# LJacksonPan/RaTrack

Hardware: AMD Instinct MI355X
Metric: radar frame-pairs/sec (backbone forward, eval) at B=64,N=256 per GPU (higher is better)
Workload: dtype f32 (2xfp16 split MFMA: three fp16 products per fp32 product, fp32 accumulate, power-of-two scales per matrix and position); 1 GPU; Track4D.backbone forward, B=64 frame-pairs x N=256 points per GPU, S=512 centroids, eval-mode BN, random-init weights, hipGraph=True, batches in flight=4; global_batch=64, parallelism=replicas x1 (no collective on the forward path)

## Files before the change

### ratrack_amd/csrc/fused_split.hip

```cpp
#include "rtk_common.h"
#include "rtk_fused.h"
#include "split_mfma.h"

namespace {

#ifndef SP_NW
#define SP_NW 4
#endif
#ifndef SP_F
#define SP_F 32
#endif
constexpr int CV_F = 32;

__global__ __launch_bounds__(256) void pack_split_kernel(int cout, int cin, const float *__restrict__ w, int transposed, u4v *__restrict__ out,
                                                         float *__restrict__ inv_scale) {
    __shared__ unsigned s_m[4];
    float m = 0.f;
    const f4 *w4 = reinterpret_cast<const f4 *>(w);
    for (int i = threadIdx.x; i < cout * cin / 4; i += 256) {
        const f4 t = w4[i];
        m = __builtin_fmaxf(__builtin_fmaxf(m, __builtin_fabsf(t.x)), __builtin_fabsf(t.y));
        m = __builtin_fmaxf(__builtin_fmaxf(m, __builtin_fabsf(t.z)), __builtin_fabsf(t.w));
    }
    unsigned mb = __float_as_uint(m);
// ... 103 lines not shown
                const unsigned bit = (a[4 * v + q][r] > 0.f ? 1u : 0u) << (4 * ((2 * v + (q >> 1)) & 7) + r);
                if (v < 4) m[q & 1].x |= bit; else m[q & 1].y |= bit;
            }
}
__device__ __forceinline__ unsigned split_mask_bits(const uint2 (&m)[2], int v, int q) {
    return ((v < 4 ? m[q & 1].x : m[q & 1].y) >> (4 * ((2 * v + (q >> 1)) & 7))) & 15u;
}

__device__ __forceinline__ f4 *cv_at(float *base, unsigned byte_off) { return reinterpret_cast<f4 *>(reinterpret_cast<char *>(base) + byte_off); }
__device__ __forceinline__ const f4 *cv_at(const float *base, unsigned byte_off) {
    return reinterpret_cast<const f4 *>(reinterpret_cast<const char *>(base) + byte_off);
}

__device__ __forceinline__ void wn_hidden(const WnSplit &W, float dx, float dy, float dz, float (&t2)[8]) {
    float t1[8];
#pragma unroll
    for (int o = 0; o < 8; ++o) {
        float a = __fmaf_rn(ldc(W.wa + o), dx, 0.f);
        a = __fmaf_rn(ldc(W.wa + 16 + o), dy, a);
        a = __fmaf_rn(ldc(W.wa + 32 + o), dz, a);
        t1[o] = fmaxf(__fadd_rn(a, ldc(W.wa + 48 + o)), 0.f);
    }
#pragma unroll
    for (int o = 0; o < 8; ++o) {
        float a = ldc(W.bb + o);
#pragma unroll
        for (int c = 0; c < 8; ++c) a = __fmaf_rn(ldc(W.wb + (16 * (c >> 2) + o) * 4 + (c & 3)), t1[c], a);
        t2[o] = fmaxf(a, 0.f);
    }
}
struct WnBlock {
    f16v bias;
    float w[4];
};
__device__ __forceinline__ WnBlock wn_block(const WnSplit &W, int v, int hh, int col) {
    WnBlock k;
    k.bias = split_bias(W.bc, v, hh);
    const int ch = 32 * v + col;
    const float *wr = W.wc + ((ch >> 4) * 64 + (ch & 15)) * 4;
#pragma unroll
    for (int st = 0; st < 4; ++st) {
        const int kk = 2 * st + hh;
        k.w[st] = ldc(wr + 64 * (kk >> 2) + (kk & 3));
    }
    return k;
}
__device__ __forceinline__ f16v wn_pre(const WnBlock &k, int hh, const float (&t2)[8]) {
    f16v w = k.bias;
#pragma unroll
    for (int st = 0; st < 4; ++st) w = mfma_f32x2(k.w[st], hh ? t2[2 * st + 1] : t2[2 * st], w);
    return w;
}
__device__ __forceinline__ float rtk_hidden_inf() {
    float v;
    asm volatile("s_mov_b32 %0, 0x7f800000" : "=s"(v));
    return v;
}
__device__ __forceinline__ float relu1(float x, float inf) { return __builtin_amdgcn_fmed3f(x, 0.f, inf); }
__device__ __forceinline__ f4 relu_med4(f4 t, float inf) { return (f4){relu1(t.x, inf), relu1(t.y, inf), relu1(t.z, inf), relu1(t.w, inf)}; }

constexpr int CV_ROWS_F4 = 32 * 32;
struct CvRowsRequest {
    const char *p2;
    f4 *rows;
    int nbrow;
    unsigned lanepart;
    int sub;
    __device__ __forceinline__ CvRowsRequest(const float *p2_, f4 *rows_, int nbrow_, int half, int lane)
        : p2(reinterpret_cast<const char *>(p2_)), rows(rows_), nbrow(nbrow_), lanepart(512u * half + (unsigned)(((lane & 31) ^ (lane >> 5)) << 4)), sub(lane >> 5) {}
    template <int T>
    __device__ __forceinline__ void one() const {
        const int r0 = __builtin_amdgcn_readlane(nbrow, 2 * T), r1 = __builtin_amdgcn_readlane(nbrow, 2 * T + 1);
        const unsigned off = ((unsigned)(sub ? r1 : r0) << 10) + (lanepart ^ (unsigned)(((2 * T) & 15) << 4));
        __builtin_amdgcn_global_load_lds((const __attribute__((address_space(1))) void *)(p2 + off),
                                         (__attribute__((address_space(3))) void *)(rows + T * 64), 16, 0, 0);
    }
    template <int... T>
    __device__ __forceinline__ void all(std::integer_sequence<int, T...>) const { (one<T>(), ...); }
};
template <int HALF>
__device__ __forceinline__ void cv_rows_request(const float *p2, int nbrow, f4 *rows, int lane) {
    asm volatile("s_waitcnt lgkmcnt(0)" ::: "memory");
    CvRowsRequest(p2, rows, nbrow, HALF, lane).all(std::make_integer_sequence<int, 16>{});
}
template <bool SAVE>
struct CvLayer2Side {
    StoreRowsSide st;
    CvRowsRequest rq;
    template <int GI>
    __device__ __forceinline__ void at(const f4 (&h)[32]) const {
        if constexpr (SAVE) st.template at<GI>(h);
        constexpr int per_chunk = CV_F / SPLIT_GF, ig = split_issue_groups(CV_F), g = GI % per_chunk, n = (GI / per_chunk) * ig + g;
        if constexpr (g < ig && 3 * n < 16) {
            rq.template one<3 * n>();
            if constexpr (3 * n + 1 < 16) rq.template one<3 * n + 1>();
            if constexpr (3 * n + 2 < 16) rq.template one<3 * n + 2>();
        }
    }
};
template <int HALF>
__device__ __forceinline__ void cv_rows_read(const f4 *rows, int col, int hh, f4 (&h)[32]) {
#pragma unroll
    for (int e = 0; e < 16; ++e) h[16 * HALF + e] = rows[col * 32 + ((2 * e + hh) ^ (col & 15))];
}
template <int K>
__device__ __forceinline__ f4 add_row_bcast(const f4 q, const f4 r) {
    f4 o;
    asm("s_nop 1\n"
        "v_add_f32_dpp %0, %4, %8 row_newbcast:%12 row_mask:0xf bank_mask:0xf\n"
        "v_add_f32_dpp %1, %5, %9 row_newbcast:%12 row_mask:0xf bank_mask:0xf\n"
        "v_add_f32_dpp %2, %6, %10 row_newbcast:%12 row_mask:0xf bank_mask:0xf\n"
        "v_add_f32_dpp %3, %7, %11 row_newbcast:%12 row_mask:0xf bank_mask:0xf"
        : "=&v"(o.x), "=&v"(o.y), "=&v"(o.z), "=&v"(o.w)
        : "v"(q.x), "v"(q.y), "v"(q.z), "v"(q.w), "v"(r.x), "v"(r.y), "v"(r.z), "v"(r.w), "n"(K));
    return o;
}
template <int K>
__device__ __forceinline__ f4 mul_row_bcast(const f4 q, const f4 r) {
    f4 o;
    asm("s_nop 1\n"
        "v_mul_f32_dpp %0, %4, %8 row_newbcast:%12 row_mask:0xf bank_mask:0xf\n"
        "v_mul_f32_dpp %1, %5, %9 row_newbcast:%12 row_mask:0xf bank_mask:0xf\n"
        "v_mul_f32_dpp %2, %6, %10 row_newbcast:%12 row_mask:0xf bank_mask:0xf\n"
        "v_mul_f32_dpp %3, %7, %11 row_newbcast:%12 row_mask:0xf bank_mask:0xf"
        : "=&v"(o.x), "=&v"(o.y), "=&v"(o.z), "=&v"(o.w)
        : "v"(q.x), "v"(q.y), "v"(q.z), "v"(q.w), "v"(r.x), "v"(r.y), "v"(r.z), "v"(r.w), "n"(K));
    return o;
}
__device__ __forceinline__ f4 add4_rn(const f4 a, const f4 b) {
    return (f4){__fadd_rn(a.x, b.x), __fadd_rn(a.y, b.y), __fadd_rn(a.z, b.z), __fadd_rn(a.w, b.w)};
}
template <int V0, int V1>
__device__ __forceinline__ void cv_layer1_blocks(const CvSplitParams &P, const f4 q0, const f4 q1, float b0, float b1, int hh, int col, float kinf, f4 (&h)[32]) {
    static_assert(V1 <= 8, "eight 32-channel blocks");
    auto block = [&](auto vc) {
        constexpr int v = decltype(vc)::value;
        f16v c;
        auto slot = [&](auto qc) {
            constexpr int q = decltype(qc)::value, e = 4 * v + q;
            const f4 t = add_row_bcast<e & 15>(e < 16 ? q0 : q1, h[e]);
            c[4 * q] = t.x; c[4 * q + 1] = t.y; c[4 * q + 2] = t.z; c[4 * q + 3] = t.w;
        };
        slot(std::integral_constant<int, 0>{}); slot(std::integral_constant<int, 1>{});
        slot(std::integral_constant<int, 2>{}); slot(std::integral_constant<int, 3>{});
        const int ch = 32 * v + col;
        const float *wr = P.wd + (ch >> 4) * 64 + (ch & 15);
        c = mfma_f32x2(ldc(wr + 16 * hh), b0, c);
        c = mfma_f32x2(ldc(wr + 16 * (2 + hh)), b1, c);
#pragma unroll
        for (int q = 0; q < 4; ++q) h[4 * v + q] = leaky_med4((f4){c[4 * q], c[4 * q + 1], c[4 * q + 2], c[4 * q + 3]}, kinf);
    };
    block(std::integral_constant<int, V0>{}); block(std::integral_constant<int, V0 + 1>{});
    block(std::integral_constant<int, V0 + 2>{}); block(std::integral_constant<int, V0 + 3>{});
}

#ifndef CV_FWD_VGPRS
#define CV_FWD_VGPRS 448
#endif
template <bool SAVE>
__global__ __launch_bounds__(64 * SP_NW) __attribute__((amdgpu_waves_per_eu(1, 1), amdgpu_num_vgpr(CV_FWD_VGPRS)))
void cost_volume_split_kernel(const CvSplitParams P) {
    const float kinf = rtk_hidden_inf();
    __shared__ __attribute__((aligned(16))) f4 s_w[2 * CV_F * 64];
    __shared__ __attribute__((aligned(16))) f4 s_rows[SP_NW * CV_ROWS_F4];
    const int lane = threadIdx.x & 63, wave = __builtin_amdgcn_readfirstlane(threadIdx.x >> 6), hh = lane >> 5, col = lane & 31, pp = col >> 4,
              j = col & 15;
    f4 *rows = s_rows + wave * CV_ROWS_F4;
    constexpr int PPW = 2 * SP_NW;
    const int groups = (P.n1 + PPW - 1) / PPW;
    const bool flat = P.gx > 0;
    const int xcd = blockIdx.x & 7, t0 = flat ? (int)(blockIdx.x >> 3) : (int)blockIdx.x, tstep = flat ? P.gx >> 3 : (int)gridDim.x;
    const int ntiles = flat ? (P.samples >> 3) * groups : groups;
    auto locate = [&](int t, int &b_, int &G_) {
        if (flat) { const int sk = t / groups; b_ = sk * 8 + xcd; G_ = t - sk * groups; }
        else { b_ = blockIdx.y; G_ = t; }
    };
    int b, bx;
    locate(t0 < ntiles ? t0 : 0, b, bx);
    WStreamA<SP_NW, CV_F, 2 * SPLIT_NF> ws;
    ws.start_parts(P.blob, s_w, wave, lane);
    const float wi2 = ldc(P.wsc), wi3 = ldc(P.wsc + 1);
    int pt = bx * PPW + 2 * wave + pp;
    bool valid = pt < P.n1;
    long i = (long)b * P.n1 + (valid ? pt : P.n1 - 1);
    long nb = 0;
    float dx = 0.f, dy = 0.f, dz = 0.f;
    f4 q0 = {0.f, 0.f, 0.f, 0.f}, q1 = q0;
    if (t0 < ntiles) {
        nb = (long)b * P.n2 + (long)P.knn[i * 16 + j];
        cv_rows_request<0>(P.p2, (int)nb, rows, lane);
        q0 = ldc4(P.p1 + i * 256 + 4 * hh + 8 * j); q1 = ldc4(P.p1 + i * 256 + 4 * hh + 8 * (16 + j));
        if (P.st) { q0 = add4_rn(q0, ldc4(P.st + b * 256 + 4 * hh + 8 * j)); q1 = add4_rn(q1, ldc4(P.st + b * 256 + 4 * hh + 8 * (16 + j))); }
        dx = __fsub_rn(P.xyz2[nb * 3], P.xyz1[i * 3]); dy = __fsub_rn(P.xyz2[nb * 3 + 1], P.xyz1[i * 3 + 1]);
        dz = __fsub_rn(P.xyz2[nb * 3 + 2], P.xyz1[i * 3 + 2]);
    }
    for (int t = t0; t < ntiles; t += tstep) {
        asm volatile("" ::: "memory");
        const bool more = t + tstep < ntiles;
        int bn, Gn;
        locate(more ? t + tstep : t, bn, Gn);
        const int ptn = Gn * PPW + 2 * wave + pp;
        const bool validn = ptn < P.n1;
        const long in_ = (long)bn * P.n1 + (validn ? ptn : P.n1 - 1);
        long knn_next = 0;
        if (more) knn_next = (long)P.knn[in_ * 16 + j];
        f4 h[32];
        float t2[8];
        {
            const float b0 = hh ? dy : dx, b1 = hh ? 0.f : dz;
            cv_rows_read<0>(rows, col, hh, h);
            cv_rows_request<1>(P.p2, (int)nb, rows, lane);
            cv_layer1_blocks<0, 4>(P, q0, q1, b0, b1, hh, col, kinf, h);
            wn_hidden(P.wn, dx, dy, dz, t2);
            __builtin_amdgcn_sched_barrier(0);
            cv_rows_read<1>(rows, col, hh, h);
            cv_layer1_blocks<4, 8>(P, q0, q1, b0, b1, hh, col, kinf, h);
        }
        const long nbn = (long)bn * P.n2 + knn_next;
        const long pos = i * 16 + j;
        const unsigned ro = (unsigned)pos * 1024u + 16u * hh;
        if (SAVE && valid) {
            uint2 m[2];
            split_sign_masks(h, m);
            P.mk1[pos * 4 + hh] = m[0];
            P.mk1[pos * 4 + 2 + hh] = m[1];
        }
        f16v acc[SPLIT_VB];
        f4 bq[2][8];
        LaneScale sc = lane_scale32(h);
        if (SAVE && P.amax) tensor_amax_update(P.amax, sc.mb);
        split_layer<0>(ws, h, sc.s, acc, SidePair<CvLayer2Side<SAVE>, BiasSide>{{StoreRowsSide{P.sv1, ro, valid}, CvRowsRequest(P.p2, rows, (int)nbn, 0, lane)},
                                                                              BiasSide{P.bias2 + 4 * hh, bq}});
        float c = sc.inv * wi2;
        split_epilogue(acc, P.bias2 + 4 * hh, bq, [&](int e, f4 a, f4 b) { h[e] = leaky_med4(scale_bias4(a, c, b), kinf); });
        if (SAVE && valid) {
            uint2 m[2];
            split_sign_masks(h, m);
            P.mk2[pos * 4 + hh] = m[0];
            P.mk2[pos * 4 + 2 + hh] = m[1];
        }
        sc = lane_scale32(h);
        if (SAVE && P.amax) tensor_amax_update(P.amax + 1, sc.mb);
        if (SAVE) split_layer<SPLIT_NF>(ws, h, sc.s, acc, SidePair<StoreRowsSide, BiasSide>{StoreRowsSide{P.sv2, ro, valid}, BiasSide{P.bias3 + 4 * hh, bq}});
        else split_layer<SPLIT_NF>(ws, h, sc.s, acc, BiasSide{P.bias3 + 4 * hh, bq});
        ws.sync();
        c = sc.inv * wi3;
        split_epilogue(acc, P.bias3 + 4 * hh, bq, [&](int e, f4 a, f4 b) { h[e] = leaky_med4(scale_bias4(a, c, b), kinf); });
        if (SAVE && valid) {
#pragma unroll
            for (int e = 0; e < 32; ++e) *cv_at(P.sv3, ro + 32u * e) = h[e];
        }
        WnBlock wk = wn_block(P.wn, 0, hh, col);
        float *o = P.out + i * P.out_pitch + 4 * hh;
        f16v wpre = wn_pre(wk, hh, t2);
        wk = wn_block(P.wn, 1, hh, col);
        auto out_block = [&](int v) {
            const f16v w = wpre;
            if (v + 1 < SPLIT_VB) wpre = wn_pre(wk, hh, t2);
            if (v + 2 < SPLIT_VB) wk = wn_block(P.wn, v + 2, hh, col);
            f4 r[4];
#pragma unroll
            for (int q = 0; q < 4; ++q)
#pragma unroll
                for (int e = 0; e < 4; ++e) r[q][e] = relu1(w[4 * q + e], kinf) * h[4 * v + q][e];
            const f4 t = row_sum16_transpose4(r[0], r[1], r[2], r[3]);
            if (valid && (j & 3) == 0) *reinterpret_cast<f4 *>(o + 32 * v + 8 * (2 * ((j >> 3) & 1) + ((j >> 2) & 1))) = t;
        };
        out_block(0);
        out_block(1);
        float cn[6] = {0.f, 0.f, 0.f, 0.f, 0.f, 0.f};
        f4 q0n = q0, q1n = q1, s0n = q0, s1n = q1;
        if (more) {
#pragma unroll
            for (int c = 0; c < 3; ++c) { cn[c] = ldc(P.xyz2 + nbn * 3 + c); cn[3 + c] = ldc(P.xyz1 + in_ * 3 + c); }
            q0n = ldc4(P.p1 + in_ * 256 + 4 * hh + 8 * j); q1n = ldc4(P.p1 + in_ * 256 + 4 * hh + 8 * (16 + j));
        }
        if (more && P.st) { s0n = ldc4(P.st + bn * 256 + 4 * hh + 8 * j); s1n = ldc4(P.st + bn * 256 + 4 * hh + 8 * (16 + j)); }
#pragma unroll
        for (int v = 2; v < SPLIT_VB; ++v) out_block(v);
        pt = ptn; valid = validn; i = in_; nb = nbn; q0 = q0n; q1 = q1n;
        if (P.st) { q0 = add4_rn(q0n, s0n); q1 = add4_rn(q1n, s1n); }
        dx = __fsub_rn(cn[0], cn[3]); dy = __fsub_rn(cn[1], cn[4]); dz = __fsub_rn(cn[2], cn[5]);
    }
    ws.finish();
}

struct CvSplitBwdParams {
    CvSplitParams f;
    const float *dout;
    int dout_pitch;
    const float *a3;
    const uint2 *mk1, *mk2;
    float *dz1, *dz2, *dz3, *dq3, *d4, *dp1, *dpd, *dt2, *dbrows;
};

__device__ __forceinline__ f4 leaky_grad_bits4(f4 d, unsigned bits) {
    return (f4){(bits & 1u) ? d.x : 0.1f * d.x, (bits & 2u) ? d.y : 0.1f * d.y, (bits & 4u) ? d.z : 0.1f * d.z, (bits & 8u) ? d.w : 0.1f * d.w};
}

__global__ __launch_bounds__(64 * SP_NW) __attribute__((amdgpu_waves_per_eu(1, 1))) void cost_volume_bwd_split_kernel(const CvSplitBwdParams Q) {
    const float kinf = rtk_hidden_inf();
    __shared__ __attribute__((aligned(16))) f4 s_w[2 * SP_F * 64];
    __shared__ float s_wct[128 * 64];
    const CvSplitParams &P = Q.f;
    const int lane = threadIdx.x & 63, wave = __builtin_amdgcn_readfirstlane(threadIdx.x >> 6), hh = lane >> 5, col = lane & 31, pp = col >> 4,
              j = col & 15;
    const int jq = 2 * ((j >> 3) & 1) + ((j >> 2) & 1);
    for (int e = threadIdx.x; e < 128 * 64; e += 64 * SP_NW) {
        const int l = e & 63, st = e >> 6, o = l & 31, ch = 32 * (st >> 4) + 8 * ((st >> 2) & 3) + 4 * (l >> 5) + (st & 3);
        s_wct[e] = o < 8 ? P.wn.wc[((ch >> 4) * 64 + (o >> 2) * 16 + (ch & 15)) * 4 + (o & 3)] : 0.f;
    }
    int b, bx, nbx;
    rtk_decode_block(P.gx, b, bx, nbx);
    constexpr int PPW = 2 * SP_NW;
    const int groups = (P.n1 + PPW - 1) / PPW;
    WStreamA<SP_NW, SP_F, 2 * SPLIT_NF> ws;
    ws.start_parts(P.blob, s_w, wave, lane);
    const float wi3 = ldc(P.wsc), wi2 = ldc(P.wsc + 1);
    int pt = bx * PPW + 2 * wave + pp;
    bool valid = pt < P.n1;
    long i = (long)b * P.n1 + (valid ? pt : P.n1 - 1);
    float dx = 0.f, dy = 0.f, dz = 0.f;
    if (bx < groups) {
        const long nb = (long)b * P.n2 + (long)P.knn[i * 16 + j];
        dx = __fsub_rn(P.xyz2[nb * 3], P.xyz1[i * 3]); dy = __fsub_rn(P.xyz2[nb * 3 + 1], P.xyz1[i * 3 + 1]);
        dz = __fsub_rn(P.xyz2[nb * 3 + 2], P.xyz1[i * 3 + 2]);
    }
    for (int G = bx; G < groups; G += nbx) {
        asm volatile("" ::: "memory");
        const long pos = i * 16 + j;
        const unsigned ro = (unsigned)pos * 1024u + 16u * hh;
        if (valid && hh == 0) *reinterpret_cast<f4 *>(Q.d4 + pos * 4) = (f4){dx, dy, dz, 1.0f};
        uint2 m2[2] = {Q.mk2[pos * 4 + hh], Q.mk2[pos * 4 + 2 + hh]}, m1[2] = {Q.mk1[pos * 4 + hh], Q.mk1[pos * 4 + 2 + hh]};
        f4 h[32];
#pragma unroll
        for (int e = 0; e < 32; ++e) h[e] = *cv_at(Q.a3, ro + 32u * e);
        float t2[8];
        WnBlock wk = wn_block(P.wn, 0, hh, col);
        const float *dor = Q.dout + i * Q.dout_pitch + 4 * hh;
        const f4 dq0 = ldc4(dor + 8 * j), dq1 = ldc4(dor + 8 * (16 + j));
        wn_hidden(P.wn, dx, dy, dz, t2);
        f16v dt2;
#pragma unroll
        for (int e = 0; e < 16; ++e) dt2[e] = 0.f;
        f16v wpre = wn_pre(wk, hh, t2);
        wk = wn_block(P.wn, 1, hh, col);
        auto block_a = [&](auto vc) {
            constexpr int v = decltype(vc)::value;
            const f16v w = wpre;
            if constexpr (v + 1 < SPLIT_VB) wpre = wn_pre(wk, hh, t2);
            if constexpr (v + 2 < SPLIT_VB) wk = wn_block(P.wn, v + 2, hh, col);
            f4 zs[4];
            auto slot = [&](auto qc) {
                constexpr int q = decltype(qc)::value, e = 4 * v + q;
                const f4 a = h[e];
                f4 wv;
#pragma unroll
                for (int r = 0; r < 4; ++r) wv[r] = relu1(w[4 * q + r], kinf);
                const f4 da = mul_row_bcast<e & 15>(e < 16 ? dq0 : dq1, a);
                const f4 t = mul_row_bcast<e & 15>(e < 16 ? dq0 : dq1, wv);
                f4 qq, z;
#pragma unroll
                for (int r = 0; r < 4; ++r) {
                    qq[r] = wv[r] > 0.f ? da[r] : 0.f;
                    z[r] = a[r] > 0.f ? t[r] : 0.1f * t[r];
                    dt2 = mfma_f32x2(s_wct[(16 * v + 4 * q + r) * 64 + lane], qq[r], dt2);
                }
                h[e] = z;
                zs[q] = z;
                if (valid) *cv_at(Q.dq3, ro + 32u * e) = qq;
            };
            slot(std::integral_constant<int, 0>{}); slot(std::integral_constant<int, 1>{});
            slot(std::integral_constant<int, 2>{}); slot(std::integral_constant<int, 3>{});
            if (Q.dbrows) {
                const f4 r = row_sum16_transpose4(zs[0], zs[1], zs[2], zs[3]);
                if (valid && (j & 3) == 0) *reinterpret_cast<f4 *>(Q.dbrows + i * 512 + 32 * v + 8 * jq + 4 * hh) = r;
            }
        };
        block_a(std::integral_constant<int, 0>{}); block_a(std::integral_constant<int, 1>{}); block_a(std::integral_constant<int, 2>{});
        block_a(std::integral_constant<int, 3>{}); block_a(std::integral_constant<int, 4>{}); block_a(std::integral_constant<int, 5>{});
        block_a(std::integral_constant<int, 6>{}); block_a(std::integral_constant<int, 7>{});
        if (valid) *reinterpret_cast<f4 *>(Q.dt2 + pos * 8 + 4 * hh) = (f4){dt2[0], dt2[1], dt2[2], dt2[3]};
        f16v acc[SPLIT_VB];
        LaneScale sc = lane_scale32(h);
        if (P.amax) tensor_amax_update(P.amax, sc.mb);
        split_layer<0>(ws, h, sc.s, acc, StoreRowsSide{Q.dz3, ro, valid});
        float c = sc.inv * wi3;
#pragma unroll
        for (int v = 0; v < SPLIT_VB; ++v) {
#pragma unroll
            for (int q = 0; q < 4; ++q) h[4 * v + q] = leaky_grad_bits4(acc_slot(acc, 4 * v + q) * c, split_mask_bits(m2, v, q));
            if (Q.dbrows) {
                const f4 r = row_sum16_transpose4(h[4 * v], h[4 * v + 1], h[4 * v + 2], h[4 * v + 3]);
                if (valid && (j & 3) == 0) *reinterpret_cast<f4 *>(Q.dbrows + i * 512 + 256 + 32 * v + 8 * jq + 4 * hh) = r;
            }
        }
        sc = lane_scale32(h);
        if (P.amax) tensor_amax_update(P.amax + 1, sc.mb);
        split_layer<SPLIT_NF>(ws, h, sc.s, acc, StoreRowsSide{Q.dz2, ro, valid});
        ws.sync();
        c = sc.inv * wi2;
        const int Gn = G + nbx;
        const bool more = Gn < groups;
        const int ptn = Gn * PPW + 2 * wave + pp;
        const bool validn = ptn < P.n1;
        const long in_ = (long)b * P.n1 + (validn ? ptn : P.n1 - 1);
        long knn_next = 0;
        if (more) knn_next = (long)P.knn[in_ * 16 + j];
        float dxn = 0.f, dyn = 0.f, dzn = 0.f;
        float *dpr = Q.dp1 + i * 256 + 4 * hh;
        float *dpd = Q.dpd + i * 768 + 4 * hh;
#pragma unroll
        for (int v = 0; v < SPLIT_VB; ++v) {
            if (v == 2 && more) {
                const long nbn = (long)b * P.n2 + knn_next;
                dxn = __fsub_rn(P.xyz2[nbn * 3], P.xyz1[in_ * 3]); dyn = __fsub_rn(P.xyz2[nbn * 3 + 1], P.xyz1[in_ * 3 + 1]);
                dzn = __fsub_rn(P.xyz2[nbn * 3 + 2], P.xyz1[in_ * 3 + 2]);
            }
            f4 r[4];
#pragma unroll
            for (int q = 0; q < 4; ++q) {
                r[q] = leaky_grad_bits4(acc_slot(acc, 4 * v + q) * c, split_mask_bits(m1, v, q));
                if (valid) *cv_at(Q.dz1, ro + 32u * (4 * v + q)) = r[q];
            }
            const f4 s0 = row_sum16_transpose4(r[0], r[1], r[2], r[3]);
            const f4 sx = row_sum16_transpose4(r[0] * dx, r[1] * dx, r[2] * dx, r[3] * dx);
            const f4 sy = row_sum16_transpose4(r[0] * dy, r[1] * dy, r[2] * dy, r[3] * dy);
            const f4 sz = row_sum16_transpose4(r[0] * dz, r[1] * dz, r[2] * dz, r[3] * dz);
            if (valid && (j & 3) == 0) {
                *reinterpret_cast<f4 *>(dpr + 32 * v + 8 * jq) = s0;
                *reinterpret_cast<f4 *>(dpd + 32 * v + 8 * jq) = sx;
                *reinterpret_cast<f4 *>(dpd + 256 + 32 * v + 8 * jq) = sy;
// ... 284 lines not shown
```

### ratrack_amd/csrc/split_mfma.h

```cpp
#pragma once
#include "fused_common.h"

typedef float f16v __attribute__((ext_vector_type(16)));

__device__ __forceinline__ f16v mfma_h(u4v a, u4v b, f16v c) {
    return __builtin_amdgcn_mfma_f32_32x32x16_f16(__builtin_bit_cast(h8v, a), __builtin_bit_cast(h8v, b), c, 0, 0, 0);
}

__device__ __forceinline__ f16v mfma_bf(u4v a, u4v b, f16v c) {
    return __builtin_amdgcn_mfma_f32_32x32x16_bf16(__builtin_bit_cast(bf8v, a), __builtin_bit_cast(bf8v, b), c, 0, 0, 0);
}

__device__ __forceinline__ LaneScale lane_scale32_of(float m) {
    const unsigned mb = __float_as_uint(m);
    const auto r = __builtin_amdgcn_permlane32_swap(mb, mb, false, false);
    return lane_scale_of(r[0] > r[1] ? r[0] : r[1]);
}
template <int N>
__device__ __forceinline__ LaneScale lane_scale32(const f4 (&h)[N]) { return lane_scale32_of(abs_max_f4(h)); }

template <int W>
__device__ __forceinline__ void split2_word_of(const f4 x0, const f4 x1, float s, u4v (&b)[2]) {
    const float xa = W < 2 ? x0[2 * W] : x1[2 * W - 4], xb = W < 2 ? x0[2 * W + 1] : x1[2 * W - 3];
    const SplitWord w = split2_word(xa, xb, s);
    b[0][W] = w.h; b[1][W] = w.l;
}

constexpr int SPLIT_GF = 4;
constexpr int split_issue_groups(int F) { return F >= 16 ? F / 16 : 1; }
constexpr int SPLIT_KS = 16;
constexpr int SPLIT_VB = 8;
constexpr int SPLIT_NF = SPLIT_KS * SPLIT_VB * 2;

template <int NW, int F, int NF>
struct WStreamA : WStream<NW, F, NF> {
    using Base = WStream<NW, F, NF>;
    unsigned rd;
    unsigned next_off;
    __device__ __forceinline__ void set_rd() {
        rd = (unsigned)(size_t)(__attribute__((address_space(3))) void *)(this->lds) + (unsigned)((this->buf * F) * 64 + this->lane) * 16u;
        const int nxt = this->cur + 1 == Base::NCHUNKS ? 0 : this->cur + 1;
        next_off = (unsigned)nxt * (unsigned)(F * 1024);
    }
    __device__ __forceinline__ void start(const f4 *blob_, f4 *lds_, int wave_, int lane_) { Base::start(blob_, lds_, wave_, lane_); set_rd(); }
    __device__ __forceinline__ void next() { Base::next(); set_rd(); }
    __device__ __forceinline__ void sync() {
        asm volatile("s_waitcnt vmcnt(0)" ::: "memory");
        __syncthreads();
        this->buf ^= 1;
        this->cur = this->cur + 1 == Base::NCHUNKS ? 0 : this->cur + 1;
        asm volatile("" : "+s"(this->cur));
        set_rd();
    }
    template <int K, int PARTS>
    __device__ __forceinline__ void issue_part() {
        static_assert(NF % F == 0, "whole chunks only");
        const char *base = this->blob + next_off;
#pragma unroll
        for (int i = K; i < (F + NW - 1) / NW; i += PARTS) {
            const int f = this->wave + i * NW;
            if (F % NW == 0 || f < F)
                __builtin_amdgcn_global_load_lds((const __attribute__((address_space(1))) void *)(base + (size_t)i * NW * 1024 + this->lane_off),
                                                 (__attribute__((address_space(3))) void *)(this->lds + ((this->buf ^ 1) * F + f) * 64), 16, 0, 0);
        }
    }
    __device__ __forceinline__ void start_parts(const f4 *blob_, f4 *lds_, int wave_, int lane_) {
        this->lds = lds_; this->wave = wave_; this->lane = lane_;
        this->blob = reinterpret_cast<const char *>(blob_);
        this->lane_off = (unsigned)(wave_ * 64 + lane_) * 16u;
        this->cur = 0; this->buf = 0;
        Base::issue(0, 0);
        asm volatile("s_waitcnt vmcnt(0)" ::: "memory");
        __syncthreads();
        set_rd();
    }
    template <int FI>
    __device__ __forceinline__ f4 frag_async() const {
        f4 r;
        asm volatile("ds_read_b128 %0, %1 offset:%2" : "=v"(r) : "v"(rd), "n"(FI * 1024));
        return r;
    }
};

template <int OUTSTANDING>
__device__ __forceinline__ void lds_wait(f4 (&c)[SPLIT_GF]) {
    asm volatile("s_waitcnt lgkmcnt(%4)" : "+v"(c[0]), "+v"(c[1]), "+v"(c[2]), "+v"(c[3]) : "n"(OUTSTANDING));
}

struct NoSide {
    template <int GI>
    __device__ __forceinline__ void at(const f4 (&)[32]) const {}
};
struct StoreRowsSide {
    float *base;
    unsigned ro;
    bool valid;
    template <int GI>
    __device__ __forceinline__ void at(const f4 (&h)[32]) const {
        if constexpr ((GI & 1) == 0) {
            if (valid) *reinterpret_cast<f4 *>(reinterpret_cast<char *>(base) + (ro + 32u * (GI / 2))) = h[GI / 2];
        }
    }
};
__device__ __forceinline__ float ldc(const float *p) { return *(const __attribute__((address_space(4))) float *)p; }
__device__ __forceinline__ f4 ldc4(const float *p) { return *(const __attribute__((address_space(4))) f4 *)p; }

__device__ __forceinline__ f4 bias_slot(const float *bias4hh, int e) {
    return *reinterpret_cast<const f4 *>(bias4hh + 32 * (e >> 2) + 8 * (e & 3));
}
struct BiasSide {
    const float *bias;
    f4 (&bq)[2][8];
    template <int GI>
    __device__ __forceinline__ void at(const f4 (&)[32]) const {
        constexpr int NG = SPLIT_KS * (SPLIT_VB / 2);
        if constexpr (GI >= NG - 4) {
            bq[0][2 * (GI - (NG - 4))] = bias_slot(bias, 2 * (GI - (NG - 4)));
            bq[0][2 * (GI - (NG - 4)) + 1] = bias_slot(bias, 2 * (GI - (NG - 4)) + 1);
        }
    }
};
template <class Emit>
__device__ __forceinline__ void split_epilogue(const f16v (&acc)[SPLIT_VB], const float *bias4hh, f4 (&bq)[2][8], Emit &&emit) {
#pragma unroll
    for (int k = 0; k < 4; ++k) {
        if (k < 3) {
#pragma unroll
            for (int e = 0; e < 8; ++e) bq[(k + 1) & 1][e] = bias_slot(bias4hh, 8 * (k + 1) + e);
        }
#pragma unroll
        for (int e = 0; e < 8; ++e) {
            const int v = (8 * k + e) >> 2, q = e & 3;
            emit(8 * k + e, (f4){acc[v][4 * q], acc[v][4 * q + 1], acc[v][4 * q + 2], acc[v][4 * q + 3]}, bq[k & 1][e]);
        }
        __builtin_amdgcn_sched_barrier(0);
    }
}
template <class A, class B>
struct SidePair {
    A a;
    B b;
    template <int GI>
    __device__ __forceinline__ void at(const f4 (&h)[32]) const { a.template at<GI>(h); b.template at<GI>(h); }
};

template <int FBASE, int GI, class WS, int F, bool ZERO>
struct SplitStep {
    static constexpr int NG = SPLIT_KS * (SPLIT_VB / 2);
    template <int GJ, int PART>
    static __device__ __forceinline__ void load_part(WS &ws, f4 (&dst)[SPLIT_GF]) {
        constexpr int f0 = FBASE + GJ * SPLIT_GF;
        if constexpr (PART == 0) {
            if constexpr (f0 % F == 0 && f0 != 0) ws.sync();
            if constexpr ((f0 % F) / SPLIT_GF < split_issue_groups(F)) ws.template issue_part<(f0 % F) / SPLIT_GF, split_issue_groups(F)>();
        }
        dst[2 * PART] = ws.template frag_async<(f0 + 2 * PART) % F>();
        dst[2 * PART + 1] = ws.template frag_async<(f0 + 2 * PART + 1) % F>();
    }
    template <int GJ>
    static __device__ __forceinline__ void load(WS &ws, f4 (&dst)[SPLIT_GF]) {
        load_part<GJ, 0>(ws, dst);
        load_part<GJ, 1>(ws, dst);
    }
    template <class Side>
    static __device__ __forceinline__ void run(WS &ws, const f4 (&h)[32], float scale, f16v (&acc)[SPLIT_VB], f4 (&a)[2][SPLIT_GF], u4v (&b)[2][2],
                                               const Side &side) {
        constexpr int s = GI / 4, v0 = (GI % 4) * 2;
        static_assert(F % SPLIT_GF == 0, "a group step reads four consecutive fragments of one chunk");
        lds_wait<0>(a[GI & 1]);
        const f4(&c)[SPLIT_GF] = a[GI & 1];
        const u4v(&B)[2] = b[s & 1];
        f16v z0, z1;
        if constexpr (ZERO && s == 0) {
#pragma unroll
            for (int e = 0; e < 16; ++e) z0[e] = z1[e] = 0.f;
        } else {
            z0 = acc[v0]; z1 = acc[v0 + 1];
        }
        acc[v0] = mfma_h(__builtin_bit_cast(u4v, c[1]), B[0], z0);
        acc[v0 + 1] = mfma_h(__builtin_bit_cast(u4v, c[3]), B[0], z1);
        if constexpr (GI + 1 < NG) load_part<GI + 1, 0>(ws, a[(GI + 1) & 1]);
        __builtin_amdgcn_sched_barrier(0);
        acc[v0] = mfma_h(__builtin_bit_cast(u4v, c[0]), B[1], acc[v0]);
        acc[v0 + 1] = mfma_h(__builtin_bit_cast(u4v, c[2]), B[1], acc[v0 + 1]);
        if constexpr (GI + 1 < NG) load_part<GI + 1, 1>(ws, a[(GI + 1) & 1]);
        __builtin_amdgcn_sched_barrier(0);
        if constexpr (s + 1 < SPLIT_KS) split2_word_of<GI % 4>(h[2 * (s + 1)], h[2 * (s + 1) + 1], scale, b[(s + 1) & 1]);
        acc[v0] = mfma_h(__builtin_bit_cast(u4v, c[0]), B[0], acc[v0]);
        acc[v0 + 1] = mfma_h(__builtin_bit_cast(u4v, c[2]), B[0], acc[v0 + 1]);
        side.template at<GI>(h);
#pragma unroll
        for (int k = 0; k < 2; ++k) {
            __builtin_amdgcn_sched_group_barrier(0x008, 1, 0);
            __builtin_amdgcn_sched_group_barrier(0x002, 3, 0);
        }
        __builtin_amdgcn_sched_barrier(0);
    }
};

template <int FBASE, class WS, int F, bool ZERO, class Side, int... GI>
__device__ __forceinline__ void split_layer_impl(WS &ws, const f4 (&h)[32], float scale, f16v (&acc)[SPLIT_VB], const Side &side,
                                                 std::integer_sequence<int, GI...>) {
    f4 a[2][SPLIT_GF];
    u4v b[2][2];
    SplitStep<FBASE, 0, WS, F, ZERO>::template load<0>(ws, a[0]);
    split2(h[0], h[1], scale, b[0]);
    __builtin_amdgcn_sched_barrier(0);
    (SplitStep<FBASE, GI, WS, F, ZERO>::run(ws, h, scale, acc, a, b, side), ...);
}

template <int FBASE, bool ZERO = true, int NW, int F, int NF, class Side = NoSide>
__device__ __forceinline__ void split_layer(WStreamA<NW, F, NF> &ws, const f4 (&h)[32], float scale, f16v (&acc)[SPLIT_VB], const Side &side = Side()) {
    split_layer_impl<FBASE, WStreamA<NW, F, NF>, F, ZERO, Side>(ws, h, scale, acc, side, std::make_integer_sequence<int, SPLIT_KS * (SPLIT_VB / 2)>{});
}

__device__ __forceinline__ f16v split_bias(const float *__restrict__ bias, int v, int hh) {
    f16v o;
#pragma unroll
    for (int q = 0; q < 4; ++q) {
        const f4 t = ldc4(bias + 32 * v + 8 * q + 4 * hh);
        o[4 * q] = t.x; o[4 * q + 1] = t.y; o[4 * q + 2] = t.z; o[4 * q + 3] = t.w;
    }
    return o;
}
__device__ __forceinline__ f4 acc_slot(const f16v (&acc)[SPLIT_VB], int e) {
    const int v = e >> 2, q = e & 3;
    return (f4){acc[v][4 * q], acc[v][4 * q + 1], acc[v][4 * q + 2], acc[v][4 * q + 3]};
}
```

Baseline: 105,500 frame-pairs/s.

## Interleave layer-3 epilogue and output reduction into layer-3 MFMA steps in eval cost volume

In the non-SAVE (eval) cost-volume kernel, layer 3 now runs in a reordered step order that finishes output column blocks early. Each block's bias, leaky activation, weight-net MFMA, product and row reduction are then interleaved slot by slot with the remaining split-MFMA steps. This replaces the serial epilogue and out_block pass. Next-tile loads are issued mid-layer, and the weight stream gains a gather addressing mode so the layer-3 weight chunks arrive in the new step order. This aims to hide epilogue VALU, cross-lane reduction and global-load latency under MFMA work, at the cost of much more complex scheduling and possible register pressure.

Result: no change. 105,200 frame-pairs/s (-0.2%).

```diff
diff --git a/ratrack_amd/csrc/fused_split.hip b/ratrack_amd/csrc/fused_split.hip
--- a/ratrack_amd/csrc/fused_split.hip
+++ b/ratrack_amd/csrc/fused_split.hip
@@ -279,6 +279,148 @@
     };
     block(std::integral_constant<int, V0>{}); block(std::integral_constant<int, V0 + 1>{});
     block(std::integral_constant<int, V0 + 2>{}); block(std::integral_constant<int, V0 + 3>{});
+}
+
+struct CvOutSide {
+    const CvSplitParams &P;
+    const float (&t2)[8];
+    const float *bias;
+    float *o;
+    float c, kinf;
+    int hh, col, j;
+    bool valid;
+    long nbn, in_;
+    int bn;
+    float (&cn)[6];
+    f4 &q0n, &q1n, &s0n, &s1n;
+    WnBlock wk;
+    f4 bs[4];
+    f16v w;
+    f4 a3[4], r[4];
+
+    template <int V>
+    __device__ __forceinline__ void request_wn() {
+#pragma unroll
+        for (int q = 0; q < 4; ++q) {
+            const f4 t = *reinterpret_cast<const f4 *>(P.wn.bc + 32 * V + 8 * q + 4 * hh);
+            wk.bias[4 * q] = t.x; wk.bias[4 * q + 1] = t.y; wk.bias[4 * q + 2] = t.z; wk.bias[4 * q + 3] = t.w;
+        }
+        const int ch = 32 * V + col;
+        const float *wr = P.wn.wc + ((ch >> 4) * 64 + (ch & 15)) * 4;
+#pragma unroll
+        for (int st = 0; st < 4; ++st) {
+            const int kk = 2 * st + hh;
+            wk.w[st] = wr[64 * (kk >> 2) + (kk & 3)];
+        }
+    }
+    template <int V>
+    __device__ __forceinline__ void request_bias() {
+#pragma unroll
+        for (int q = 0; q < 4; ++q) bs[q] = bias_slot(bias, 4 * V + q);
+    }
+    __device__ __forceinline__ void take_operands() {
+        asm volatile("" : "+v"(bs[0]), "+v"(bs[1]), "+v"(bs[2]), "+v"(bs[3]), "+v"(wk.w[0]), "+v"(wk.w[1]), "+v"(wk.w[2]), "+v"(wk.w[3]));
+    }
+    template <int V, int N>
+    __device__ __forceinline__ void slot(const f16v &A) {
+        constexpr int g = N / 6, K = N % 6;
+        if constexpr (N == 0 && V > 0) take_operands();
+        if constexpr (g < 4 && K == 0) w = mfma_f32x2(wk.w[g], hh ? t2[2 * g + 1] : t2[2 * g], g == 0 ? wk.bias : w);
+        if constexpr (g < 4 && K == 2) a3[g] = scale_bias4((f4){A[4 * g], A[4 * g + 1], A[4 * g + 2], A[4 * g + 3]}, c, bs[g]);
+        if constexpr (g < 4 && K == 4) a3[g] = leaky_med4(a3[g], kinf);
+        if constexpr (g == 3 && K == 5 && V + 1 < SPLIT_VB) request_wn<V + 1>();
+        if constexpr (g == 4 && K == 5 && V + 1 < SPLIT_VB) request_bias<V + 1>();
+        if constexpr (g == 4 || (g == 5 && K < 2)) {
+            constexpr int q = g == 4 ? K / 2 : 3, e0 = 2 * (K & 1);
+#pragma unroll
+            for (int e = e0; e < e0 + 2; ++e) r[q][e] = relu1(w[4 * q + e], kinf) * a3[q][e];
+        }
+        if constexpr (g == 5 && K == 2) row_sum_pair8(r[0], r[2]);
+        if constexpr (g == 5 && K == 4) row_sum_pair8(r[1], r[3]);
+        if constexpr (g == 6 && K == 0) row_sum_pair4(r[0], r[1]);
+        if constexpr (g == 6 && K == 2) quad_sum_valu_f4(r[0]);
+        if constexpr (g == 6 && K == 4) {
+            if (valid && (j & 3) == 0) *reinterpret_cast<f4 *>(o + 32 * V + 8 * (2 * ((j >> 3) & 1) + ((j >> 2) & 1))) = r[0];
+        }
+    }
+    template <int V, int... N>
+    __device__ __forceinline__ void block(const f16v &A, std::integer_sequence<int, N...>) { (slot<V, N>(A), ...); }
+    template <int PART>
+    __device__ __forceinline__ void next_tile() {
+        if constexpr (PART == 0) {
+#pragma unroll
+            for (int k = 0; k < 3; ++k) { cn[k] = ldc(P.xyz2 + nbn * 3 + k); cn[3 + k] = ldc(P.xyz1 + in_ * 3 + k); }
+        } else if constexpr (PART == 1) {
+            q0n = ldc4(P.p1 + in_ * 256 + 4 * hh + 8 * j); q1n = ldc4(P.p1 + in_ * 256 + 4 * hh + 8 * (16 + j));
+        } else {
+            const float *sp = P.st ? P.st + (long)bn * 256 : P.p1 + in_ * 256;
+            s0n = ldc4(sp + 4 * hh + 8 * j); s1n = ldc4(sp + 4 * hh + 8 * (16 + j));
+        }
+    }
+    template <int GI, int K>
+    __device__ __forceinline__ void at(const f16v (&acc)[SPLIT_VB]) {
+        if constexpr (GI >= 16) {
+            constexpr int V = (GI - 16) / 8;
+            slot<V, ((GI - 16) % 8) * 6 + K>(acc[V]);
+            if constexpr (K == 3 && GI >= 36 && GI < 39) next_tile<GI - 36>();
+        }
+    }
+};
+
+template <int FBASE, int GI, class WS, int F>
+struct CvL3Step {
+    using Ld = SplitStep<FBASE, 0, WS, F, true>;
+    static constexpr int NG = SPLIT_KS * (SPLIT_VB / 2);
+    static __device__ __forceinline__ void run(WS &ws, const f4 (&h)[32], float scale, f16v (&acc)[SPLIT_VB], f4 (&a)[2][SPLIT_GF], u4v (&pc)[SPLIT_KS][2],
+                                               CvOutSide &side) {
+        constexpr int s = GI % SPLIT_KS, v0 = (GI / SPLIT_KS) * 2;
+        lds_wait<0>(a[GI & 1]);
+        const f4(&c)[SPLIT_GF] = a[GI & 1];
+        const u4v(&B)[2] = pc[s];
+        f16v z0, z1;
+        if constexpr (s == 0) {
+#pragma unroll
+            for (int e = 0; e < 16; ++e) z0[e] = z1[e] = 0.f;
+        } else {
+            z0 = acc[v0]; z1 = acc[v0 + 1];
+        }
+        constexpr bool split = GI + 1 < SPLIT_KS;
+        acc[v0] = mfma_h(__builtin_bit_cast(u4v, c[1]), B[0], z0);
+        if constexpr (split) split2_word_of<0>(h[2 * (s + 1)], h[2 * (s + 1) + 1], scale, pc[s + 1]);
+        side.template at<GI, 0>(acc);
+        __builtin_amdgcn_sched_barrier(0);
+        acc[v0 + 1] = mfma_h(__builtin_bit_cast(u4v, c[3]), B[0], z1);
+        if constexpr (GI + 1 < NG) Ld::template load_part<GI + 1, 0>(ws, a[(GI + 1) & 1]);
+        side.template at<GI, 1>(acc);
+        __builtin_amdgcn_sched_barrier(0);
+        acc[v0] = mfma_h(__builtin_bit_cast(u4v, c[0]), B[1], acc[v0]);
+        if constexpr (split) split2_word_of<1>(h[2 * (s + 1)], h[2 * (s + 1) + 1], scale, pc[s + 1]);
+        side.template at<GI, 2>(acc);
+        __builtin_amdgcn_sched_barrier(0);
+        acc[v0 + 1] = mfma_h(__builtin_bit_cast(u4v, c[2]), B[1], acc[v0 + 1]);
+        if constexpr (GI + 1 < NG) Ld::template load_part<GI + 1, 1>(ws, a[(GI + 1) & 1]);
+        side.template at<GI, 3>(acc);
+        __builtin_amdgcn_sched_barrier(0);
+        acc[v0] = mfma_h(__builtin_bit_cast(u4v, c[0]), B[0], acc[v0]);
+        if constexpr (split) split2_word_of<2>(h[2 * (s + 1)], h[2 * (s + 1) + 1], scale, pc[s + 1]);
+        side.template at<GI, 4>(acc);
+        __builtin_amdgcn_sched_barrier(0);
+        acc[v0 + 1] = mfma_h(__builtin_bit_cast(u4v, c[2]), B[0], acc[v0 + 1]);
+        if constexpr (split) split2_word_of<3>(h[2 * (s + 1)], h[2 * (s + 1) + 1], scale, pc[s + 1]);
+        side.template at<GI, 5>(acc);
+        __builtin_amdgcn_sched_barrier(0);
+    }
+};
+template <int FBASE, int G0, class WS, int F, int... GI>
+__device__ __forceinline__ void cv_layer3_steps(WS &ws, const f4 (&h)[32], float scale, f16v (&acc)[SPLIT_VB], f4 (&a)[2][SPLIT_GF], u4v (&pc)[SPLIT_KS][2],
+                                                CvOutSide &side, std::integer_sequence<int, GI...>) {
+    (CvL3Step<FBASE, G0 + GI, WS, F>::run(ws, h, scale, acc, a, pc, side), ...);
+}
+template <int FBASE, class WS, int F>
+__device__ __forceinline__ void cv_layer3_start(WS &ws, const f4 (&h)[32], float scale, f4 (&a)[2][SPLIT_GF], u4v (&pc)[SPLIT_KS][2]) {
+    SplitStep<FBASE, 0, WS, F, true>::template load<0>(ws, a[0]);
+    split2(h[0], h[1], scale, pc[0]);
+    __builtin_amdgcn_sched_barrier(0);
 }
 
 #ifndef CV_FWD_VGPRS
@@ -304,7 +446,8 @@
     };
     int b, bx;
     locate(t0 < ntiles ? t0 : 0, b, bx);
-    WStreamA<SP_NW, CV_F, 2 * SPLIT_NF> ws;
+    using WS = WStreamA<SP_NW, CV_F, 2 * SPLIT_NF, SAVE ? -1 : SPLIT_NF / CV_F>;
+    WS ws;
     ws.start_parts(P.blob, s_w, wave, lane);
     const float wi2 = ldc(P.wsc), wi3 = ldc(P.wsc + 1);
     int pt = bx * PPW + 2 * wave + pp;
@@ -358,6 +501,11 @@
         if (SAVE && P.amax) tensor_amax_update(P.amax, sc.mb);
         split_layer<0>(ws, h, sc.s, acc, SidePair<CvLayer2Side<SAVE>, BiasSide>{{StoreRowsSide{P.sv1, ro, valid}, CvRowsRequest(P.p2, rows, (int)nbn, 0, lane)},
                                                                               BiasSide{P.bias2 + 4 * hh, bq}});
+        float cn[6] = {0.f, 0.f, 0.f, 0.f, 0.f, 0.f};
+        f4 q0n = q0, q1n = q1, s0n = q0, s1n = q1;
+        float *o = P.out + i * P.out_pitch + 4 * hh;
+        CvOutSide side{P, t2, P.bias3 + 4 * hh, o, 0.f, kinf, hh, col, j, valid, nbn, in_, bn, cn, q0n, q1n, s0n, s1n};
+        if constexpr (!SAVE) { side.template request_wn<0>(); side.template request_bias<0>(); }
         float c = sc.inv * wi2;
         split_epilogue(acc, P.bias2 + 4 * hh, bq, [&](int e, f4 a, f4 b) { h[e] = leaky_med4(scale_bias4(a, c, b), kinf); });
         if (SAVE && valid) {
@@ -368,43 +516,52 @@
         }
         sc = lane_scale32(h);
         if (SAVE && P.amax) tensor_amax_update(P.amax + 1, sc.mb);
-        if (SAVE) split_layer<SPLIT_NF>(ws, h, sc.s, acc, SidePair<StoreRowsSide, BiasSide>{StoreRowsSide{P.sv2, ro, valid}, BiasSide{P.bias3 + 4 * hh, bq}});
-        else split_layer<SPLIT_NF>(ws, h, sc.s, acc, BiasSide{P.bias3 + 4 * hh, bq});
-        ws.sync();
-        c = sc.inv * wi3;
-        split_epilogue(acc, P.bias3 + 4 * hh, bq, [&](int e, f4 a, f4 b) { h[e] = leaky_med4(scale_bias4(a, c, b), kinf); });
-        if (SAVE && valid) {
-#pragma unroll
-            for (int e = 0; e < 32; ++e) *cv_at(P.sv3, ro + 32u * e) = h[e];
-        }
-        WnBlock wk = wn_block(P.wn, 0, hh, col);
-        float *o = P.out + i * P.out_pitch + 4 * hh;
-        f16v wpre = wn_pre(wk, hh, t2);
-        wk = wn_block(P.wn, 1, hh, col);
-        auto out_block = [&](int v) {
-            const f16v w = wpre;
-            if (v + 1 < SPLIT_VB) wpre = wn_pre(wk, hh, t2);
-            if (v + 2 < SPLIT_VB) wk = wn_block(P.wn, v + 2, hh, col);
-            f4 r[4];
-#pragma unroll
-            for (int q = 0; q < 4; ++q)
-#pragma unroll
-                for (int e = 0; e < 4; ++e) r[q][e] = relu1(w[4 * q + e], kinf) * h[4 * v + q][e];
-            const f4 t = row_sum16_transpose4(r[0], r[1], r[2], r[3]);
-            if (valid && (j & 3) == 0) *reinterpret_cast<f4 *>(o + 32 * v + 8 * (2 * ((j >> 3) & 1) + ((j >> 2) & 1))) = t;
-        };
-        out_block(0);
-        out_block(1);
-        float cn[6] = {0.f, 0.f, 0.f, 0.f, 0.f, 0.f};
-        f4 q0n = q0, q1n = q1, s0n = q0, s1n = q1;
-        if (more) {
-#pragma unroll
-            for (int c = 0; c < 3; ++c) { cn[c] = ldc(P.xyz2 + nbn * 3 + c); cn[3 + c] = ldc(P.xyz1 + in_ * 3 + c); }
-            q0n = ldc4(P.p1 + in_ * 256 + 4 * hh + 8 * j); q1n = ldc4(P.p1 + in_ * 256 + 4 * hh + 8 * (16 + j));
-        }
-        if (more && P.st) { s0n = ldc4(P.st + bn * 256 + 4 * hh + 8 * j); s1n = ldc4(P.st + bn * 256 + 4 * hh + 8 * (16 + j)); }
-#pragma unroll
-        for (int v = 2; v < SPLIT_VB; ++v) out_block(v);
+        if constexpr (SAVE) {
+            split_layer<SPLIT_NF>(ws, h, sc.s, acc, SidePair<StoreRowsSide, BiasSide>{StoreRowsSide{P.sv2, ro, valid}, BiasSide{P.bias3 + 4 * hh, bq}});
+            ws.sync();
+            c = sc.inv * wi3;
+            split_epilogue(acc, P.bias3 + 4 * hh, bq, [&](int e, f4 a, f4 b) { h[e] = leaky_med4(scale_bias4(a, c, b), kinf); });
+            if (valid) {
+#pragma unroll
+                for (int e = 0; e < 32; ++e) *cv_at(P.sv3, ro + 32u * e) = h[e];
+            }
+            WnBlock wk = wn_block(P.wn, 0, hh, col);
+            f16v wpre = wn_pre(wk, hh, t2);
+            wk = wn_block(P.wn, 1, hh, col);
+            auto out_block = [&](int v) {
+                const f16v w = wpre;
+                if (v + 1 < SPLIT_VB) wpre = wn_pre(wk, hh, t2);
+                if (v + 2 < SPLIT_VB) wk = wn_block(P.wn, v + 2, hh, col);
+                f4 r[4];
+#pragma unroll
+                for (int q = 0; q < 4; ++q)
+#pragma unroll
+                    for (int e = 0; e < 4; ++e) r[q][e] = relu1(w[4 * q + e], kinf) * h[4 * v + q][e];
+                const f4 t = row_sum16_transpose4(r[0], r[1], r[2], r[3]);
+                if (valid && (j & 3) == 0) *reinterpret_cast<f4 *>(o + 32 * v + 8 * (2 * ((j >> 3) & 1) + ((j >> 2) & 1))) = t;
+            };
+            out_block(0);
+            out_block(1);
+            if (more) {
+#pragma unroll
+                for (int c = 0; c < 3; ++c) { cn[c] = ldc(P.xyz2 + nbn * 3 + c); cn[3 + c] = ldc(P.xyz1 + in_ * 3 + c); }
+                q0n = ldc4(P.p1 + in_ * 256 + 4 * hh + 8 * j); q1n = ldc4(P.p1 + in_ * 256 + 4 * hh + 8 * (16 + j));
+            }
+            if (more && P.st) { s0n = ldc4(P.st + bn * 256 + 4 * hh + 8 * j); s1n = ldc4(P.st + bn * 256 + 4 * hh + 8 * (16 + j)); }
+#pragma unroll
+            for (int v = 2; v < SPLIT_VB; ++v) out_block(v);
+        } else {
+            f4 a[2][SPLIT_GF];
+            u4v pc[SPLIT_KS][2];
+            side.c = sc.inv * wi3;
+            side.take_operands();
+            cv_layer3_start<SPLIT_NF, WS, CV_F>(ws, h, sc.s, a, pc);
+            cv_layer3_steps<SPLIT_NF, 0, WS, CV_F>(ws, h, sc.s, acc, a, pc, side, std::make_integer_sequence<int, SPLIT_KS>{});
+            cv_layer3_steps<SPLIT_NF, SPLIT_KS, WS, CV_F>(ws, h, sc.s, acc, a, pc, side, std::make_integer_sequence<int, 3 * SPLIT_KS>{});
+            ws.sync();
+            side.template block<6>(acc[6], std::make_integer_sequence<int, 48>{});
+            side.template block<7>(acc[7], std::make_integer_sequence<int, 48>{});
+        }
         pt = ptn; valid = validn; i = in_; nb = nbn; q0 = q0n; q1 = q1n;
         if (P.st) { q0 = add4_rn(q0n, s0n); q1 = add4_rn(q1n, s1n); }
         dx = __fsub_rn(cn[0], cn[3]); dy = __fsub_rn(cn[1], cn[4]); dz = __fsub_rn(cn[2], cn[5]);
diff --git a/ratrack_amd/csrc/split_mfma.h b/ratrack_amd/csrc/split_mfma.h
--- a/ratrack_amd/csrc/split_mfma.h
+++ b/ratrack_amd/csrc/split_mfma.h
@@ -32,15 +32,23 @@
 constexpr int SPLIT_VB = 8;
 constexpr int SPLIT_NF = SPLIT_KS * SPLIT_VB * 2;
 
-template <int NW, int F, int NF>
+template <int NW, int F, int NF, int GATHER = -1>
 struct WStreamA : WStream<NW, F, NF> {
     using Base = WStream<NW, F, NF>;
+    static_assert(GATHER < 0 || (NW == 4 && F % 4 == 0 && 64 % F == 0), "the gather takes one fragment of a group step per wave");
     unsigned rd;
     unsigned next_off;
+    unsigned next_stride;
     __device__ __forceinline__ void set_rd() {
         rd = (unsigned)(size_t)(__attribute__((address_space(3))) void *)(this->lds) + (unsigned)((this->buf * F) * 64 + this->lane) * 16u;
         const int nxt = this->cur + 1 == Base::NCHUNKS ? 0 : this->cur + 1;
         next_off = (unsigned)nxt * (unsigned)(F * 1024);
+        if constexpr (GATHER >= 0) {
+            constexpr int CP = 64 / F;
+            const int c = nxt - GATHER;
+            next_stride = c >= 0 ? 16u * 1024u : (unsigned)(NW * 1024);
+            if (c >= 0) next_off = (unsigned)(GATHER * F + (c % CP) * (F / 4) * 16 + 4 * (c / CP)) * 1024u;
+        }
     }
     __device__ __forceinline__ void start(const f4 *blob_, f4 *lds_, int wave_, int lane_) { Base::start(blob_, lds_, wave_, lane_); set_rd(); }
     __device__ __forceinline__ void next() { Base::next(); set_rd(); }
@@ -60,7 +68,7 @@
         for (int i = K; i < (F + NW - 1) / NW; i += PARTS) {
             const int f = this->wave + i * NW;
             if (F % NW == 0 || f < F)
-                __builtin_amdgcn_global_load_lds((const __attribute__((address_space(1))) void *)(base + (size_t)i * NW * 1024 + this->lane_off),
+                __builtin_amdgcn_global_load_lds((const __attribute__((address_space(1))) void *)(base + (GATHER >= 0 ? (size_t)((unsigned)i * next_stride) : (size_t)i * NW * 1024) + this->lane_off),
                                                  (__attribute__((address_space(3))) void *)(this->lds + ((this->buf ^ 1) * F + f) * 64), 16, 0, 0);
         }
     }
@@ -209,9 +217,9 @@
     (SplitStep<FBASE, GI, WS, F, ZERO>::run(ws, h, scale, acc, a, b, side), ...);
 }
 
-template <int FBASE, bool ZERO = true, int NW, int F, int NF, class Side = NoSide>
-__device__ __forceinline__ void split_layer(WStreamA<NW, F, NF> &ws, const f4 (&h)[32], float scale, f16v (&acc)[SPLIT_VB], const Side &side = Side()) {
-    split_layer_impl<FBASE, WStreamA<NW, F, NF>, F, ZERO, Side>(ws, h, scale, acc, side, std::make_integer_sequence<int, SPLIT_KS * (SPLIT_VB / 2)>{});
+template <int FBASE, bool ZERO = true, int NW, int F, int NF, int GATHER, class Side = NoSide>
+__device__ __forceinline__ void split_layer(WStreamA<NW, F, NF, GATHER> &ws, const f4 (&h)[32], float scale, f16v (&acc)[SPLIT_VB], const Side &side = Side()) {
+    split_layer_impl<FBASE, WStreamA<NW, F, NF, GATHER>, F, ZERO, Side>(ws, h, scale, acc, side, std::make_integer_sequence<int, SPLIT_KS * (SPLIT_VB / 2)>{});
 }
 
 __device__ __forceinline__ f16v split_bias(const float *__restrict__ bias, int v, int hh) {
```
